# guptakhil/show-tell

Hardware: AMD Instinct MI355X
Metric: training images/sec (ResNet101+GRU, emb=512, bs=128) at 1/2/4/8 MI355X (higher is better)
Workload: dtype bf16; 1 GPU; BASELINE configs[1]: ResNet-101 (train-mode BN, frozen) + 5-layer GRU decoder, E=H=512, V=10000, fwd+bwd+SGD step, synthetic COCO-shaped batch; batch_per_gpu=128, global_batch=128, image=3x224x224, parallelism=dp1

## Files before the change

### include/showtell_hip.h

```cpp
#ifndef SHOWTELL_HIP_H
#define SHOWTELL_HIP_H

#include <stddef.h>
#include <stdint.h>

#ifdef __cplusplus
extern "C" {
#endif

#define ST_F32 0
#define ST_BF16 1

#define ST_CELL_GRU 0
#define ST_CELL_LSTM 1

const char* st_last_error(void);
int st_version(void);

typedef struct {
  const void* x;
  const void* w;
  void* y;
  const float* bias;
  const float* scale;
  const float* shift;
  const void* residual;
  float* stats;
  int dtype, out_dtype;
  int B, Hin, Win, Cin, Ho, Wo, N, KH, KW, stride, pad;
  int ldx, ldw, ldy;
  int relu, accumulate;
  int Cin_logical;
  int k_order;
  int stats_replicas;
  const float* in_stats; const float* in_gamma; const float* in_beta; float in_count, in_eps;
  int split_k;
} st_conv_desc;

int st_conv(const st_conv_desc* d, void* stream);
int st_conv_batch(const st_conv_desc* d, int n, void* stream);

typedef struct {
  const void* x; const void* w_frag; void* y;
  float* stats; int stats_replicas;
  const float* scale; const float* shift; int relu;
  const float* in_stats; const float* in_gamma; const float* in_beta; float in_count; float in_eps;
  int B, H, W, C, N;
  int in_stats_replicas;
} st_conv3x3_img_desc;
int st_conv3x3_img_supported(int H, int W, int C, int N);
int st_conv3x3_img(const st_conv3x3_img_desc* d, void* stream);
int st_conv3x3_s2_supported(int C, int N);
int st_conv3x3_s2(const st_conv3x3_img_desc* d, void* stream);
typedef struct {
  const void* x; const void* w_frag; void* y; const void* residual;
  float* stats; int stats_replicas;
  const float* scale; const float* shift; int relu;
  const float* in_stats; const float* in_gamma; const float* in_beta; float in_count; float in_eps; int in_stats_replicas;
  int B, Hin, Win, C, N, stride;
} st_conv1x1_wreg_desc;
int st_conv1x1_wreg_supported(int C, int N);
int st_conv1x1_wreg(const st_conv1x1_wreg_desc* d, void* stream);
int st_conv1x1_kstream_supported(int C, int N);
int st_conv1x1_kstream(const st_conv1x1_wreg_desc* d, void* stream);
typedef struct {
  const void* raw; const void* identity; void* x_out; const void* w_frag; void* y;
  float* stats; int stats_replicas;
  const float* f_stats; const float* f_gamma; const float* f_beta; float f_count; float f_eps; int f_stats_replicas;
  long rows; int C, N;
  const float* id_stats; const float* id_gamma; const float* id_beta; int id_stats_replicas;
} st_conv1x1_kfuse_desc;
int st_conv1x1_kfuse_supported(int C, int N);
int st_conv1x1_kfuse(const st_conv1x1_kfuse_desc* d, void* stream);
#ifdef ST_EXPERIMENTAL
int st_conv1x1_kfuse8(const st_conv1x1_kfuse_desc* d, void* stream);
#endif
typedef struct {
  const void* raw2; const void* w3_frag; const void* identity; void* x_out; const void* w1_frag; void* y;
  float* stats; int stats_replicas;
  const float* bn2_stats; const float* bn2_gamma; const float* bn2_beta; int bn2_replicas;
  const float* bn3_stats; const float* bn3_gamma; const float* bn3_beta; int bn3_replicas;
  const float* id_stats; const float* id_gamma; const float* id_beta; int id_replicas;
  float count; float eps;
  long rows; int C1, C2, N;
} st_conv_b2b_desc;
int st_conv_b2b_supported(int C1, int C2, int N);
int st_conv_b2b(const st_conv_b2b_desc* d, void* stream);
typedef struct {
  const void* x2; const void* w3_frag; const void* identity; void* x_out; const void* w1_frag; void* y;
  float* stats; int stats_replicas;
  const float* bn2_stats; const float* bn2_gamma; const float* bn2_beta; int bn2_replicas;
  const float* bn3_stats; const float* bn3_gamma; const float* bn3_beta; int bn3_replicas;
  float count; float eps;
  const float* scale3; const float* shift3; const float* scale1; const float* shift1; int relu1;
  long rows; int C1, C2, N;
  const float* id_stats; const float* id_gamma; const float* id_beta; int id_replicas;
} st_conv_c3c1_desc;
int st_conv_c3c1_supported(int C1, int C2, int N);
int st_conv_c3c1(const st_conv_c3c1_desc* d, void* stream);
int st_conv1x1_astat_supported(int C, int N);
int st_conv1x1_astat(const st_conv1x1_wreg_desc* d, void* stream);

int st_pack_conv_weight_frag(const float* w, void* out, int Cout, int Cin, int KH, int KW, int ntw, void* stream);

int st_tune(int reserved, int kc, int w8);
int st_prof_enable(int on);
int st_debug_stamps(unsigned long long* buf);
int st_prof_collect(double* ms, double* flops, long* launches);

typedef struct {
  const void* x; void* y; const void* res;
  const float* stats;  const float* gamma; const float* beta;
  const float* running_mean; const float* running_var;
  const float* res_stats; const float* res_gamma; const float* res_beta;
  const float* res_running_mean; const float* res_running_var;
  int res_bn;
  int dtype; long rows; int C; float count; float eps; int relu;
  int stats_replicas, res_stats_replicas;
} st_bn_act_desc;

int st_bn_act(const st_bn_act_desc* d, void* stream);

int st_bn_update_running(const float* stats, float* running_mean, float* running_var,
// ... 288 lines not shown
```

### show-tell_amd/_lib.py

```python
import ctypes as C
import os

import torch

_HERE = os.path.dirname(os.path.abspath(__file__))
LIB_PATH = os.path.join(_HERE, "lib", "libshowtell_hip.so")

ST_F32, ST_BF16 = 0, 1
ST_CELL_GRU, ST_CELL_LSTM = 0, 1

c_p, c_i, c_f, c_l = C.c_void_p, C.c_int, C.c_float, C.c_long


class ConvDesc(C.Structure):
    _fields_ = [("x", c_p), ("w", c_p), ("y", c_p), ("bias", c_p), ("scale", c_p), ("shift", c_p),
                ("residual", c_p), ("stats", c_p), ("dtype", c_i), ("out_dtype", c_i),
                ("B", c_i), ("Hin", c_i), ("Win", c_i), ("Cin", c_i), ("Ho", c_i), ("Wo", c_i), ("N", c_i),
                ("KH", c_i), ("KW", c_i), ("stride", c_i), ("pad", c_i),
                ("ldx", c_i), ("ldw", c_i), ("ldy", c_i), ("relu", c_i), ("accumulate", c_i), ("Cin_logical", c_i), ("k_order", c_i), ("stats_replicas", c_i),
                ("in_stats", c_p), ("in_gamma", c_p), ("in_beta", c_p), ("in_count", c_f), ("in_eps", c_f), ("split_k", c_i)]


class Conv3x3ImgDesc(C.Structure):
    _fields_ = [("x", c_p), ("w_frag", c_p), ("y", c_p), ("stats", c_p), ("stats_replicas", c_i), ("scale", c_p), ("shift", c_p),
# ... 8 lines not shown


class Conv1x1KfuseDesc(C.Structure):
    _fields_ = [("raw", c_p), ("identity", c_p), ("x_out", c_p), ("w_frag", c_p), ("y", c_p), ("stats", c_p), ("stats_replicas", c_i),
                ("f_stats", c_p), ("f_gamma", c_p), ("f_beta", c_p), ("f_count", c_f), ("f_eps", c_f), ("f_stats_replicas", c_i),
                ("rows", c_l), ("C", c_i), ("N", c_i),
                ("id_stats", c_p), ("id_gamma", c_p), ("id_beta", c_p), ("id_stats_replicas", c_i)]


class StemConvPoolDesc(C.Structure):
    _fields_ = [("x_s2d", c_p), ("w_frag", c_p), ("y", c_p), ("stats", c_p), ("stats_replicas", c_i), ("gamma", c_p),
                ("scale", c_p), ("shift", c_p), ("B", c_i), ("H", c_i), ("W", c_i)]


class ConvB2bDesc(C.Structure):
    _fields_ = [("raw2", c_p), ("w3_frag", c_p), ("identity", c_p), ("x_out", c_p), ("w1_frag", c_p), ("y", c_p),
                ("stats", c_p), ("stats_replicas", c_i),
                ("bn2_stats", c_p), ("bn2_gamma", c_p), ("bn2_beta", c_p), ("bn2_replicas", c_i),
                ("bn3_stats", c_p), ("bn3_gamma", c_p), ("bn3_beta", c_p), ("bn3_replicas", c_i),
                ("id_stats", c_p), ("id_gamma", c_p), ("id_beta", c_p), ("id_replicas", c_i),
                ("count", c_f), ("eps", c_f), ("rows", c_l), ("C1", c_i), ("C2", c_i), ("N", c_i)]


class ConvC3c1Desc(C.Structure):
    _fields_ = [("x2", c_p), ("w3_frag", c_p), ("identity", c_p), ("x_out", c_p), ("w1_frag", c_p), ("y", c_p),
                ("stats", c_p), ("stats_replicas", c_i),
                ("bn2_stats", c_p), ("bn2_gamma", c_p), ("bn2_beta", c_p), ("bn2_replicas", c_i),
                ("bn3_stats", c_p), ("bn3_gamma", c_p), ("bn3_beta", c_p), ("bn3_replicas", c_i),
                ("count", c_f), ("eps", c_f),
                ("scale3", c_p), ("shift3", c_p), ("scale1", c_p), ("shift1", c_p), ("relu1", c_i),
                ("rows", c_l), ("C1", c_i), ("C2", c_i), ("N", c_i),
                ("id_stats", c_p), ("id_gamma", c_p), ("id_beta", c_p), ("id_replicas", c_i)]


class BnActDesc(C.Structure):
    _fields_ = [("x", c_p), ("y", c_p), ("res", c_p), ("stats", c_p), ("gamma", c_p), ("beta", c_p),
                ("running_mean", c_p), ("running_var", c_p), ("res_stats", c_p), ("res_gamma", c_p),
                ("res_beta", c_p), ("res_running_mean", c_p), ("res_running_var", c_p), ("res_bn", c_i),
                ("dtype", c_i), ("rows", c_l), ("C", c_i), ("count", c_f), ("eps", c_f), ("relu", c_i),
                ("stats_replicas", c_i), ("res_stats_replicas", c_i)]


ST_MAX_LAYERS = 8


class RnnParams(C.Structure):
    _fields_ = [("cell", c_i), ("dtype", c_i), ("L", c_i), ("in0", c_i), ("H", c_i), ("V", c_i), ("E", c_i),
                ("emb", c_p), ("w_ih", c_p * ST_MAX_LAYERS), ("w_hh", c_p * ST_MAX_LAYERS),
                ("b_ih", c_p * ST_MAX_LAYERS), ("b_hh", c_p * ST_MAX_LAYERS), ("w_lin", c_p), ("b_lin", c_p)]


class RnnGrads(C.Structure):
    _fields_ = [("emb", c_p), ("w_ih", c_p * ST_MAX_LAYERS), ("w_hh", c_p * ST_MAX_LAYERS),
                ("b_ih", c_p * ST_MAX_LAYERS), ("b_hh", c_p * ST_MAX_LAYERS), ("w_lin", c_p), ("b_lin", c_p)]


class AttnParams(C.Structure):
    _fields_ = [("rnn", RnnParams), ("F", c_i), ("A", c_i), ("P", c_i),
                ("w_enc", c_p), ("b_enc", c_p), ("w_dec", c_p), ("b_dec", c_p), ("w_full", c_p), ("b_full", c_p),
                ("w_init_h", c_p), ("b_init_h", c_p), ("w_init_c", c_p), ("b_init_c", c_p), ("w_embed", c_p), ("b_embed", c_p)]


class AttnGrads(C.Structure):
    _fields_ = [("rnn", RnnGrads)] + [(n, c_p) for n in ("w_enc", "b_enc", "w_dec", "b_dec", "w_full", "b_full", "w_init_h", "b_init_h",
                                                        "w_init_c", "b_init_c", "w_embed", "b_embed")]


class PackedSeq(C.Structure):
    _fields_ = [("B", c_i), ("T", c_i), ("ntok", c_i), ("Tcap", c_i), ("batch_sizes_host", C.POINTER(c_i)),
                ("rows_b", c_p), ("rows_t", c_p), ("prev_row", c_p), ("caption", c_p)]


class ImageBatchDesc(C.Structure):
    _fields_ = [("src", c_p), ("src_bytes", C.c_int64), ("offset", c_p), ("height", c_p), ("width", c_p), ("flip", c_p), ("batch", c_i),
                ("max_height", c_i), ("max_width", c_i), ("out_h", c_i), ("out_w", c_i), ("lut", c_p), ("tmp", c_p),
                ("out", c_p), ("out_u8", c_p)]


_SIGS = {
    "st_version": ([], c_i),
    "st_image_transform": ([C.POINTER(ImageBatchDesc), c_p], c_i),
    "st_conv": ([C.POINTER(ConvDesc), c_p], c_i),
    "st_conv_batch": ([C.POINTER(ConvDesc), c_i, c_p], c_i),
    "st_conv3x3_img_supported": ([c_i, c_i, c_i, c_i], c_i),
    "st_conv3x3_img": ([C.POINTER(Conv3x3ImgDesc), c_p], c_i),
    "st_conv3x3_s2_supported": ([c_i, c_i], c_i),
    "st_conv3x3_s2": ([C.POINTER(Conv3x3ImgDesc), c_p], c_i),
    "st_conv1x1_wreg_supported": ([c_i, c_i], c_i),
    "st_conv1x1_wreg": ([C.POINTER(Conv1x1WregDesc), c_p], c_i),
    "st_conv1x1_kfuse": ([C.POINTER(Conv1x1KfuseDesc), c_p], c_i),
    "st_conv1x1_kfuse_supported": ([c_i, c_i], c_i),
    "st_conv1x1_kfuse8": ([C.POINTER(Conv1x1KfuseDesc), c_p], c_i),
    "st_conv_b2b": ([C.POINTER(ConvB2bDesc), c_p], c_i),
    "st_conv_b2b_supported": ([c_i, c_i, c_i], c_i),
    "st_conv_c3c1": ([C.POINTER(ConvC3c1Desc), c_p], c_i),
    "st_conv_c3c1_supported": ([c_i, c_i, c_i], c_i),
    "st_conv1x1_astat_supported": ([c_i, c_i], c_i),
    "st_conv1x1_astat": ([C.POINTER(Conv1x1WregDesc), c_p], c_i),
    "st_conv1x1_kstream_supported": ([c_i, c_i], c_i),
    "st_conv1x1_kstream": ([C.POINTER(Conv1x1WregDesc), c_p], c_i),
    "st_pack_conv_weight_frag": ([c_p, c_p, c_i, c_i, c_i, c_i, c_i, c_p], c_i),
    "st_tune": ([c_i, c_i, c_i], c_i),
    "st_prof_enable": ([c_i], c_i),
    "st_debug_stamps": ([c_p], c_i),
    "st_prof_collect": ([C.POINTER(C.c_double), C.POINTER(C.c_double), C.POINTER(c_l)], c_i),
    "st_bn_act": ([C.POINTER(BnActDesc), c_p], c_i),
    "st_bn_update_running": ([c_p, c_p, c_p, c_i, c_f, c_f, c_p], c_i),
    "st_nchw_to_nhwc": ([c_p, c_p, c_i, c_i, c_i, c_i, c_i, c_i, c_p], c_i),
    "st_nchw_to_s2d16": ([c_p, c_p, c_i, c_i, c_i, c_i, c_p], c_i),
    "st_stem_weight_s2d": ([c_p, c_p, c_i, c_i, c_p], c_i),
    "st_stem_weight_frag": ([c_p, c_p, c_p], c_i),
    "st_stem_weight_frag_packed": ([c_p, c_i, c_p, c_p], c_i),
    "st_stem_conv_pool": ([C.POINTER(StemConvPoolDesc), c_p], c_i),
    "st_nhwc_to_ncp_f32": ([c_p, c_p, c_i, c_i, c_i, c_i, c_p], c_i),
    "st_maxpool3x3s2": ([c_p, c_p, c_i, c_i, c_i, c_i, c_i, c_p], c_i),
    "st_maxpool3x3s2_bn": ([c_p, c_p, c_i, c_i, c_i, c_i, c_i, c_p, c_p, c_p, c_p, c_p, c_f, c_f, c_p], c_i),
    "st_global_avgpool": ([c_p, c_p, c_i, c_i, c_i, c_i, c_i, c_p], c_i),
    "st_cast": ([c_p, c_p, c_i, c_i, c_l, c_p], c_i),
    "st_transpose": ([c_p, c_p, c_i, c_i, c_i, c_i, c_i, c_p], c_i),
    "st_transpose_colsum": ([c_p, c_p, c_p, c_i, c_i, c_i, c_i, c_i, c_p], c_i),
    "st_transpose_batch": ([c_p, c_p, c_p, c_i, c_i, c_i, c_i, c_i, c_i, c_p, c_p, c_p], c_i),
    "st_pack_conv_weight": ([c_p, c_p, c_i, c_i, c_i, c_i, c_i, c_i, c_i, c_p], c_i),
    "st_cast2d": ([c_p, c_p, c_i, c_i, c_i, c_i, c_i, c_i, c_p], c_i),
    "st_rnn_vocab_ld": ([c_i], c_i),
    "st_rnn_workspace_bytes": ([C.POINTER(RnnParams), C.POINTER(PackedSeq)], C.c_size_t),
    "st_rnn_forward": ([C.POINTER(RnnParams), C.POINTER(PackedSeq), c_p, c_p, c_p, C.c_size_t, c_p, c_i, c_i, c_p, c_i, c_p], c_i),
    "st_rnn_fused_loss_supported": ([C.POINTER(RnnParams)], c_i),
    "st_rnn_fused_loss_bytes": ([C.POINTER(RnnParams), C.POINTER(PackedSeq)], C.c_size_t),
    "st_rnn_fused_loss": ([C.POINTER(RnnParams), C.POINTER(PackedSeq), c_p, C.c_size_t, c_p, c_p, C.c_size_t, c_p, c_p], c_i),
    "st_rnn_fused_dlogits": ([C.POINTER(RnnParams), C.POINTER(PackedSeq), c_p, C.c_size_t, c_p, c_p, c_p, c_p, c_i, c_p], c_i),
    "st_rnn_fused_loss_w": ([C.POINTER(RnnParams), C.POINTER(PackedSeq), c_p, C.c_size_t, c_p, c_p, C.c_size_t, c_p, c_p, c_p, c_p], c_i),
    "st_rnn_fused_dlogits_w": ([C.POINTER(RnnParams), C.POINTER(PackedSeq), c_p, C.c_size_t, c_p, c_p, c_p, c_p, c_p, c_i, c_p], c_i),
    "st_rnn_fused_loss_ls_bytes": ([C.POINTER(RnnParams), C.POINTER(PackedSeq)], C.c_size_t),
    "st_rnn_fused_loss_ls": ([C.POINTER(RnnParams), C.POINTER(PackedSeq), c_p, C.c_size_t, c_p, c_p, C.c_size_t, c_p, c_p, c_p, c_f, c_p,
                             C.c_size_t, c_p, c_p], c_i),
    "st_rnn_fused_dlogits_ls": ([C.POINTER(RnnParams), C.POINTER(PackedSeq), c_p, C.c_size_t, c_p, c_p, c_p, c_p, c_f, c_p, c_i, c_p], c_i),
    "st_rnn_backward": ([C.POINTER(RnnParams), C.POINTER(RnnGrads), C.POINTER(PackedSeq), c_p, c_p, c_i, c_p, c_p, C.c_size_t,
                         c_p, c_p, c_p], c_i),
    "st_dropout_rows": ([c_p, c_p, c_i, c_i, c_i, c_i, c_i, C.c_double, c_l, c_i, c_i, c_i, c_p], c_i),
    "st_rnn_dropout_bytes": ([C.POINTER(RnnParams), C.POINTER(PackedSeq)], C.c_size_t),
    "st_rnn_forward_drop": ([C.POINTER(RnnParams), C.POINTER(PackedSeq), c_p, c_p, c_p, C.c_size_t, c_p, c_i, c_i, c_p, c_i, c_p, c_p], c_i),
    "st_rnn_fused_loss_drop": ([C.POINTER(RnnParams), C.POINTER(PackedSeq), c_p, C.c_size_t, c_p, c_p, C.c_size_t, c_p, c_p, c_p, c_f, c_p,
                               C.c_size_t, c_p, c_p, c_p], c_i),
    "st_rnn_fused_dlogits_drop": ([C.POINTER(RnnParams), C.POINTER(PackedSeq), c_p, C.c_size_t, c_p, c_p, c_p, c_p, c_f, c_p, c_i, c_p, c_p],
                                  c_i),
    "st_rnn_backward_drop": ([C.POINTER(RnnParams), C.POINTER(RnnGrads), C.POINTER(PackedSeq), c_p, c_p, c_i, c_p, c_p, C.c_size_t,
                              c_p, c_p, c_p, c_p], c_i),
    "st_rnn_forward_ids": ([C.POINTER(RnnParams), C.POINTER(PackedSeq), c_p, c_p, c_p, C.c_size_t, c_p, c_i, c_i, c_p, c_i, c_p, c_p, c_p], c_i),
    "st_rnn_backward_ids": ([C.POINTER(RnnParams), C.POINTER(RnnGrads), C.POINTER(PackedSeq), c_p, c_p, c_i, c_p, c_p, C.c_size_t,
                             c_p, c_p, c_p, c_p, c_p], c_i),
    "st_rnn_greedy_workspace_bytes": ([C.POINTER(RnnParams), c_i], C.c_size_t),
    "st_rnn_greedy": ([C.POINTER(RnnParams), c_p, c_i, c_i, c_p, C.c_size_t, c_p, c_p, c_p], c_i),
    "st_rnn_greedy_last_route": ([], c_i),
    "st_rnn_step": ([C.POINTER(RnnParams), c_p, c_i, c_p, c_p, c_p, c_p, c_p, c_i, c_p], c_i),
    "st_embedding_rows": ([c_p, c_p, c_p, c_i, c_i, c_i, c_i, c_i, c_p], c_i),
    "st_gather_state": ([c_p, c_p, c_p, c_i, c_i, c_i, c_i, c_i, c_p], c_i),
    "st_softmax_topk": ([c_p, c_i, c_i, c_i, c_i, c_p, c_p, c_i, c_p], c_i),
    "st_beam_select": ([c_p, c_p, c_p, c_p, c_p, c_i, c_i, c_i, c_l, c_p, c_p, c_p, c_p, c_p, c_p], c_i),
    "st_beam_ban_topk": ([c_p, c_i, c_i, c_i, c_i, c_p, c_i, c_i, c_i, c_p, c_i, c_l, c_i, c_p, c_p, c_p], c_i),
    "st_beam_select_hist": ([c_p, c_p, c_p, c_p, c_p, c_i, c_i, c_i, c_l, c_p, c_p, c_p, c_p, c_p, c_p, c_p, c_i, c_i, c_p], c_i),
    "st_sample_rows": ([c_p, c_i, c_i, c_i, c_p, c_i, c_f, c_i, c_l, c_p, c_p, c_p, c_i, c_i, c_p, c_p], c_i),
    "st_rnn_sample_workspace_bytes": ([C.POINTER(RnnParams), c_i], C.c_size_t),
    "st_rnn_sample": ([C.POINTER(RnnParams), c_p, c_i, c_i, c_p, c_f, c_i, c_l, c_p, C.c_size_t, c_p, c_p, c_p], c_i),
    "st_sample_mix_rows": ([c_p, c_i, c_i, c_i, c_p, c_i, c_f, c_i, c_p, c_i, c_f, c_p, c_i, c_l, c_p, c_i, c_p, c_p, c_p, c_p, c_i, c_i, c_p,
                            c_p], c_i),
    "st_rnn_sched_inputs_workspace_bytes": ([C.POINTER(RnnParams), c_i], C.c_size_t),
# ... 115 lines not shown
```

### show-tell_amd/csrc/rnn.cpp

```cpp
#include "decoder_host.h"
#include <stdlib.h>

namespace {

struct Plan {
  int G, GH, Np, Vp, maxw;
  size_t es;
  size_t x0, y, gates, cst, dyl, dx0, dgx, dgh, dhc, dcc, tA, tB, wT, wThh, wTih, gA, gB, total;
};

Plan make_plan(const st_rnn_params* p, const st_packed_seq* s) {
  Plan q;
  q.G = p->cell == ST_CELL_GRU ? 3 : 4;
  q.GH = q.G * p->H;
  q.Np = st_up8(s->ntok);
  q.Vp = st_rnn_vocab_ld(p->V);
  q.es = st_dtype_size(p->dtype);
  q.maxw = p->in0 > p->H ? p->in0 : p->H;
  const size_t n = s->ntok, L = p->L, H = p->H;
  Arena ar;
  q.x0 = ar.take(n * p->in0 * q.es);
  q.y = ar.take(L * n * H * q.es);
  q.gates = ar.take(L * n * 4 * H * q.es);
  q.cst = ar.take(p->cell == ST_CELL_LSTM ? L * n * H * q.es : 0);
// ... 184 lines not shown
  const char* ytop = reinterpret_cast<const char*>(workspace) + q.y + (size_t)(p->L - 1) * s->ntok * p->H * q.es;
  const int n = s->ntok;
  return vocab_ce_forward(ytop, p->w_lin, p->b_lin, targets, n, p->V, scratch + 2 * (size_t)n, scratch + n, scratch, loss_accum,
                          row_weight, nll_out, reinterpret_cast<hipStream_t>(stream), tile_sums, smooth_out, label_smoothing);
}
extern "C" int st_rnn_fused_dlogits_ls(const st_rnn_params* p, const st_packed_seq* s, const void* workspace, size_t workspace_bytes,
                                       const long* targets, const float* scratch, const float* grad_scale_dev, const float* row_weight,
                                       float label_smoothing, void* dlogits, int ldd, void* stream) {
  if (check_common(p, s, "st_rnn_fused_dlogits_ls")) return 1;
  ST_CHECK(workspace && targets && scratch && dlogits, "st_rnn_fused_dlogits_ls: null pointer");
  ST_CHECK(label_smoothing >= 0.f && label_smoothing < 1.f, "st_rnn_fused_dlogits_ls: label_smoothing=%g outside [0, 1)", (double)label_smoothing);
  ST_CHECK(st_rnn_fused_loss_supported(p), "st_rnn_fused_dlogits_ls: unsupported configuration");
  const Plan q = make_plan(p, s);
  ST_CHECK(workspace_bytes >= q.total, "st_rnn_fused_dlogits_ls: workspace too small");
  const char* ytop = reinterpret_cast<const char*>(workspace) + q.y + (size_t)(p->L - 1) * s->ntok * p->H * q.es;
  return vocab_ce_dlogits(ytop, p->w_lin, p->b_lin, targets, scratch, s->ntok, p->V, dlogits, ldd, 1.0f, grad_scale_dev, row_weight,
                          reinterpret_cast<hipStream_t>(stream), true, label_smoothing);
}

namespace {
int fused_rows(const st_rnn_params* p, const st_packed_seq* s, const void* workspace, size_t workspace_bytes, const st_dropout* drop,
               const char* who, const char** ytop) {
  if (check_common(p, s, who)) return 1;
  ST_CHECK(st_rnn_fused_loss_supported(p), "%s: needs bf16, H = 512 and the vocabulary projection", who);
  const Plan q = make_plan(p, s);
  ST_CHECK(workspace && workspace_bytes >= q.total, "%s: workspace too small", who);
  DropPlan dp;
  if (st_drop_plan(drop, p->L, s->ntok, p->H, p->dtype, false, who, &dp)) return 1;
  *ytop = dp.out ? dp.rows(p->L - 1) : reinterpret_cast<const char*>(workspace) + q.y + (size_t)(p->L - 1) * s->ntok * p->H * q.es;
  return 0;
}
}
extern "C" int st_rnn_fused_loss_drop(const st_rnn_params* p, const st_packed_seq* s, const void* workspace, size_t workspace_bytes,
                                      const long* targets, float* scratch, size_t scratch_bytes, const float* row_weight, float* nll_out,
                                      float* smooth_out, float label_smoothing, float* tile_sums, size_t tile_sums_bytes, float* loss_accum,
                                      const st_dropout* drop, void* stream) {
  const char* ytop;
  if (fused_rows(p, s, workspace, workspace_bytes, drop, "st_rnn_fused_loss_drop", &ytop)) return 1;
  ST_CHECK(targets && scratch && (loss_accum || nll_out || smooth_out), "st_rnn_fused_loss_drop: null pointer");
  ST_CHECK(label_smoothing >= 0.f && label_smoothing < 1.f, "st_rnn_fused_loss_drop: label_smoothing=%g outside [0, 1)", (double)label_smoothing);
  ST_CHECK(scratch_bytes >= st_rnn_fused_loss_bytes(p, s), "st_rnn_fused_loss_drop: scratch too small");
  const int n = s->ntok;
  hipStream_t st = reinterpret_cast<hipStream_t>(stream);
  if (label_smoothing == 0.f && !smooth_out)
    return vocab_ce_forward(ytop, p->w_lin, p->b_lin, targets, n, p->V, scratch + 2 * (size_t)n, scratch + n, scratch, loss_accum, row_weight,
                            nll_out, st);
  ST_CHECK(tile_sums && tile_sums_bytes >= st_rnn_fused_loss_ls_bytes(p, s), "st_rnn_fused_loss_drop: tile_sums too small");
  return vocab_ce_forward(ytop, p->w_lin, p->b_lin, targets, n, p->V, scratch + 2 * (size_t)n, scratch + n, scratch, loss_accum, row_weight,
                          nll_out, st, tile_sums, smooth_out, label_smoothing);
}
extern "C" int st_rnn_fused_dlogits_drop(const st_rnn_params* p, const st_packed_seq* s, const void* workspace, size_t workspace_bytes,
                                         const long* targets, const float* scratch, const float* grad_scale_dev, const float* row_weight,
                                         float label_smoothing, void* dlogits, int ldd, const st_dropout* drop, void* stream) {
  const char* ytop;
  if (fused_rows(p, s, workspace, workspace_bytes, drop, "st_rnn_fused_dlogits_drop", &ytop)) return 1;
  ST_CHECK(targets && scratch && dlogits, "st_rnn_fused_dlogits_drop: null pointer");
  ST_CHECK(label_smoothing >= 0.f && label_smoothing < 1.f, "st_rnn_fused_dlogits_drop: label_smoothing=%g outside [0, 1)", (double)label_smoothing);
  return vocab_ce_dlogits(ytop, p->w_lin, p->b_lin, targets, scratch, s->ntok, p->V, dlogits, ldd, 1.0f, grad_scale_dev, row_weight,
                          reinterpret_cast<hipStream_t>(stream), label_smoothing != 0.f, label_smoothing);
}

namespace {
int rnn_backward(const st_rnn_params* p, const st_rnn_grads* g, const st_packed_seq* s,
                 const void* x0_override, const void* dlogits, int ldd, const float* dy_top_extra,
                 void* workspace, size_t workspace_bytes, float* dfeat, float* dx0_out, const st_dropout* drop, const long* input_ids, void* stream) {
  if (check_common(p, s, "st_rnn_backward")) return 1;
  ST_CHECK(g && workspace, "st_rnn_backward: null pointer");
  DropPlan dp;
  if (st_drop_plan(drop, p->L, s->ntok, p->H, p->dtype, false, "st_rnn_backward", &dp)) return 1;
  ST_CHECK(!(dp.in && x0_override), "st_rnn_backward: input dropout needs the call's own x0 rows (no x0_override)");
  ST_CHECK(!(dp.out && !dlogits), "st_rnn_backward: p_out masks the gradient of the vocabulary projection (needs dlogits, not dy_top)");
  const Plan q = make_plan(p, s);
  ST_CHECK(workspace_bytes >= q.total, "st_rnn_backward: workspace too small (%zu < %zu)", workspace_bytes, q.total);
  hipStream_t st = reinterpret_cast<hipStream_t>(stream);
  char* ws = reinterpret_cast<char*>(workspace);
  const int dt = p->dtype, H = p->H, n = s->ntok, Np = q.Np, GH = q.GH;
  const size_t es = q.es;
  const std::vector<int> off = st_packed_offsets(s);
  const int L = p->L, T = s->T;
  auto dyl = [&](int l) { return reinterpret_cast<float*>(ws + q.dyl) + (size_t)l * n * H; };
  float* dy = dyl(L - 1);
  const char* ytop = dp.out ? dp.rows(L - 1) : ws + q.y + (size_t)(p->L - 1) * n * H * es;

  if (dlogits) {
    ST_CHECK(p->w_lin && g->w_lin && g->b_lin, "st_rnn_backward: vocabulary projection gradients requested without buffers");
    ST_CHECK(ldd >= st_up8(p->V) && ldd % 8 == 0 && ldd <= q.Vp, "st_rnn_backward: dlogits leading dimension %d must be a multiple of 8 in [%d, %d]",
             ldd, st_up8(p->V), q.Vp);
    if (st_transpose_colsum(dlogits, ws + q.tA, g->b_lin, dt, n, p->V, ldd, Np, stream)) return 1;
    if (st_transpose(ytop, ws + q.tB, dt, n, H, H, Np, stream)) return 1;
    if (st_gemm_nt(ws + q.tA, Np, ws + q.tB, Np, g->w_lin, H, p->V, H, Np, dt, ST_F32, nullptr, stream, 1)) return 1;
    if (st_transpose(p->w_lin, ws + q.wT, dt, p->V, H, H, ldd, stream)) return 1;
    const int bk = dt == ST_BF16 ? 64 : 32;
    const int split = (ldd % (8 * bk) == 0 && ldd >= 16 * bk) ? 8 : 0;
    if (st_gemm_nt(dlogits, ldd, ws + q.wT, ldd, dy, H, n, H, ldd, dt, ST_F32, nullptr, stream, 0, split)) return 1;
    if (dy_top_extra) { st_set_error("st_rnn_backward: dlogits and dy_top_extra are exclusive"); return 1; }
    if (dp.out && dropout_rows_launch(dy, dy, ST_F32, n, H, H, H, dp.kout, L - 1, 0, st)) return 1;
  } else {
    ST_CHECK(dy_top_extra, "st_rnn_backward: need dlogits or dy_top");
    if (hipMemcpyAsync(dy, dy_top_extra, (size_t)n * H * sizeof(float), hipMemcpyDeviceToDevice, st) != hipSuccess) {
      st_set_error("st_rnn_backward: copy failed"); return 1;
    }
  }

  const void* x0 = x0_override ? x0_override : ws + q.x0;
  const bool need_dx0 = dfeat || dx0_out || g->emb;
  float* dx0 = dx0_out ? dx0_out : reinterpret_cast<float*>(ws + q.dx0);
  const bool gru = p->cell == ST_CELL_GRU;
  auto dgxl = [&](int l) { return ws + q.dgx + (size_t)l * n * GH * es; };
  auto dghl = [&](int l) { return gru ? ws + q.dgh + (size_t)l * n * GH * es : dgxl(l); };
  auto dhcl = [&](int l) { return reinterpret_cast<float*>(ws + q.dhc) + (size_t)l * s->B * H; };
  auto dccl = [&](int l) { return reinterpret_cast<float*>(ws + q.dcc) + (size_t)l * s->B * H; };
  auto wThh = [&](int l) { return ws + q.wThh + (size_t)l * H * GH * es; };
  auto wTih = [&](int l) { return ws + q.wTih + (size_t)l * q.maxw * GH * es; };
  if (hipMemsetAsync(ws + q.dhc, 0, (size_t)L * s->B * H * sizeof(float), st) != hipSuccess ||
      hipMemsetAsync(ws + q.dcc, 0, (size_t)L * s->B * H * sizeof(float), st) != hipSuccess) { st_set_error("memset failed"); return 1; }
  {
    const void* wx[2][ST_MAX_LAYERS]; void* wy[2][ST_MAX_LAYERS];
    int ni = 0;
    for (int l = 0; l < L; ++l) {
      const int in = l == 0 ? p->in0 : H;
      wx[0][l] = p->w_hh[l]; wy[0][l] = wThh(l);
      if (!(l > 0 || need_dx0)) continue;
      if (in == H) { wx[1][ni] = p->w_ih[l]; wy[1][ni] = wTih(l); ++ni; }
      else if (st_transpose(p->w_ih[l], wTih(l), dt, GH, in, in, GH, stream)) return 1;
    }
    if (st_transpose_batch(wx[0], wy[0], nullptr, L, dt, GH, H, H, GH, nullptr, nullptr, stream)) return 1;
    if (ni && st_transpose_batch(wx[1], wy[1], nullptr, ni, dt, GH, H, H, GH, nullptr, nullptr, stream)) return 1;
  }
  auto bwd_cell = [&](int l, int t, const float* dyrows) {
    const char* yl = ws + q.y + (size_t)l * n * H * es;
    const char* gl = ws + q.gates + (size_t)l * n * 4 * H * es;
    const char* cl = ws + q.cst + (size_t)l * n * H * es;
    RnnBwdCell c;
    memset(&c, 0, sizeof(c));
    c.dy = dyrows ? dyrows + (size_t)off[t] * H : nullptr; c.dhc = dhcl(l); c.dcc = dccl(l);
    c.cache = gl + (size_t)off[t] * 4 * H * es;
    c.hprev = t > 0 ? yl + (size_t)off[t - 1] * H * es : nullptr;
    c.cnew = cl + (size_t)off[t] * H * es;
    c.cprev = t > 0 ? cl + (size_t)off[t - 1] * H * es : nullptr;
    c.dgx = dgxl(l) + (size_t)off[t] * GH * es; c.dgh = dghl(l) + (size_t)off[t] * GH * es; c.Bt = s->batch_sizes_host[t];
    return c;
  };
  const char* env = getenv("ST_BPTT_FUSED");
  const bool fused = !(env && env[0] == '0') || dp.layer;
  for (int d = T + L - 2; fused && d >= 0; --d) {
    RnnBwdFused fc[ST_MAX_LAYERS];
    RnnDropArgs da;
    memset(&da, 0, sizeof(da));
    da.key = dp.klayer;
    int nf = 0;
    for (int l = d < T ? 0 : d - (T - 1); l <= d && l < L; ++l) {
      const int t = d - l;
      RnnBwdFused& f = fc[nf++];
      memset(&f, 0, sizeof(f));
      f.e = bwd_cell(l, t, l == L - 1 ? dy : nullptr);
      da.site[nf - 1] = l; da.row0[nf - 1] = off[t];
      RnnGemmArgs& a = f.g;
      a.M = f.e.Bt; a.N = H;
      if (t + 1 < T) {
        a.A = dghl(l) + (size_t)off[t + 1] * GH * es; a.W = wThh(l); a.M2 = s->batch_sizes_host[t + 1]; a.K = GH; a.lda = GH; a.ldw = GH;
      }
      if (l + 1 < L) {
        a.A2 = dgxl(l + 1) + (size_t)off[t] * GH * es; a.W2 = wTih(l + 1); a.K2 = GH; a.lda2 = GH; a.ldw2 = GH;
      }
    }
    if (dp.layer ? rnn_bwd_fused_launch_batch_drop(fc, nf, p->cell, dt, da, st) : rnn_bwd_fused_launch_batch(fc, nf, p->cell, dt, st)) return 1;
  }
  if (fused && need_dx0 && st_gemm_nt(dgxl(0), GH, wTih(0), GH, dx0, p->in0, n, p->in0, GH, dt, ST_F32, nullptr, stream)) return 1;
  for (int d = T + L - 2; !fused && d >= 0; --d) {
    RnnBwdCell gc[ST_MAX_LAYERS];
    RnnGemmArgs mc[2 * ST_MAX_LAYERS];
    int ng = 0, nm = 0;
    for (int l = d < T ? 0 : d - (T - 1); l <= d && l < L; ++l) {
      const int t = d - l;
      const int bt = s->batch_sizes_host[t];
      const int in = l == 0 ? p->in0 : H;
      gc[ng++] = bwd_cell(l, t, dyl(l));
      if (t > 0) {
        RnnGemmArgs& a = mc[nm++];
        memset(&a, 0, sizeof(a));
        a.A = dghl(l) + (size_t)off[t] * GH * es; a.W = wThh(l); a.M = bt; a.N = H; a.K = GH; a.lda = GH; a.ldw = GH;
        a.out_f32 = dhcl(l); a.ldo = H; a.accumulate = 1;
      }
      if (l > 0 || need_dx0) {
        RnnGemmArgs& a = mc[nm++];
        memset(&a, 0, sizeof(a));
        a.A = dgxl(l) + (size_t)off[t] * GH * es; a.W = wTih(l); a.M = bt; a.N = in; a.K = GH; a.lda = GH; a.ldw = GH;
        a.out_f32 = (l > 0 ? dyl(l - 1) + (size_t)off[t] * H : dx0 + (size_t)off[t] * in); a.ldo = in;
      }
    }
    if (rnn_bwd_gates_launch_batch(gc, ng, H, p->cell, dt, st)) return 1;
    if (rnn_gemm_launch_batch(mc, nm, dt, 0, 0, st)) return 1;
  }
  if (dp.in && need_dx0 && dropout_rows_launch(dx0, dx0, ST_F32, n, p->in0, p->in0, p->in0, dp.kin, kDropSiteInput, 0, st)) return 1;
  st_conv_desc gd[2 * ST_MAX_LAYERS];
  int ng = 0;
  auto wgrad = [&](const void* aT, const void* bT, float* dw, int rows, int cols) {
    gd[ng++] = st_gemm_nt_desc(aT, Np, bT, Np, dw, cols, rows, cols, Np, dt, ST_F32, nullptr, 1);
  };
  const void* tx[4][ST_MAX_LAYERS]; void* ty[4][ST_MAX_LAYERS]; float* tc[4][ST_MAX_LAYERS];
  int nx = 0;
  for (int l = 0; l < L; ++l) {
    const int in = l == 0 ? p->in0 : H;
    const char* xl = l == 0 ? reinterpret_cast<const char*>(x0) : dp.layer ? dp.rows(l - 1) : ws + q.y + (size_t)(l - 1) * n * H * es;
    char* aIh = ws + q.gA + (size_t)(2 * l) * GH * Np * es;
    char* aHh = ws + q.gA + (size_t)(2 * l + 1) * GH * Np * es;
    char* bIh = ws + q.gB + (size_t)(2 * l) * q.maxw * Np * es;
    char* bHh = ws + q.gB + (size_t)(2 * l + 1) * q.maxw * Np * es;
    tx[0][l] = dgxl(l); ty[0][l] = aIh; tc[0][l] = g->b_ih[l];
    tx[2][l] = dghl(l); ty[2][l] = aHh; tc[2][l] = g->b_hh[l];
    tx[3][l] = ws + q.y + (size_t)l * n * H * es; ty[3][l] = bHh; tc[3][l] = nullptr;
    if (in == H) {
      tx[1][nx] = xl; ty[1][nx] = bIh; tc[1][nx] = nullptr; ++nx;
      wgrad(aIh, bIh, g->w_ih[l], GH, in);
    } else {
      if (st_transpose(xl, bIh, dt, n, in, in, Np, stream)) return 1;
    }
    wgrad(gru ? aHh : aIh, bHh, g->w_hh[l], GH, H);
    if (!gru && colsum_launch(dghl(l), g->b_hh[l], n, GH, GH, dt, st)) return 1;
  }
  if (st_transpose_batch(tx[0], ty[0], tc[0], L, dt, n, GH, GH, Np, nullptr, nullptr, stream)) return 1;
  if (nx && st_transpose_batch(tx[1], ty[1], nullptr, nx, dt, n, H, H, Np, nullptr, nullptr, stream)) return 1;
  if (gru && st_transpose_batch(tx[2], ty[2], tc[2], L, dt, n, GH, GH, Np, nullptr, nullptr, stream)) return 1;
  if (st_transpose_batch(tx[3], ty[3], nullptr, L, dt, n, H, H, Np, s->rows_t, s->prev_row, stream)) return 1;
  for (int l = 0; l < L; ++l) {
    const int in = l == 0 ? p->in0 : H;
    if (in != H && st_gemm_nt(ws + q.gA + (size_t)(2 * l) * GH * Np * es, Np, ws + q.gB + (size_t)(2 * l) * q.maxw * Np * es, Np,
                              g->w_ih[l], in, GH, in, Np, dt, ST_F32, nullptr, stream, 1)) return 1;
  }
  for (int i = 0; i < ng; i += 12) {
    if (st_conv_batch(gd + i, ng - i < 12 ? ng - i : 12, stream)) return 1;
  }
  if (need_dx0 && !x0_override) {
    ST_CHECK(g->emb, "st_rnn_backward: embedding gradient buffer missing");
    if (embedding_bwd_launch(dx0, input_ids ? input_ids : s->caption, s->Tcap, s->rows_b, s->rows_t, dfeat, g->emb, n, p->E, p->V, 0, st)) return 1;
  }
  return 0;
}
}

extern "C" int st_rnn_backward(const st_rnn_params* p, const st_rnn_grads* g, const st_packed_seq* s,
                               const void* x0_override, const void* dlogits, int ldd, const float* dy_top_extra,
                               void* workspace, size_t workspace_bytes, float* dfeat, float* dx0_out, void* stream) {
  return rnn_backward(p, g, s, x0_override, dlogits, ldd, dy_top_extra, workspace, workspace_bytes, dfeat, dx0_out, nullptr, nullptr, stream);
}
extern "C" int st_rnn_backward_drop(const st_rnn_params* p, const st_rnn_grads* g, const st_packed_seq* s,
                                    const void* x0_override, const void* dlogits, int ldd, const float* dy_top_extra,
                                    void* workspace, size_t workspace_bytes, float* dfeat, float* dx0_out, const st_dropout* drop,
                                    void* stream) {
  return rnn_backward(p, g, s, x0_override, dlogits, ldd, dy_top_extra, workspace, workspace_bytes, dfeat, dx0_out, drop, nullptr, stream);
}
extern "C" int st_rnn_backward_ids(const st_rnn_params* p, const st_rnn_grads* g, const st_packed_seq* s,
                                   const void* x0_override, const void* dlogits, int ldd, const float* dy_top_extra,
                                   void* workspace, size_t workspace_bytes, float* dfeat, float* dx0_out, const st_dropout* drop,
                                   const long* input_ids, void* stream) {
  ST_CHECK(!(input_ids && x0_override), "st_rnn_backward_ids: input_ids and x0_override are exclusive");
  return rnn_backward(p, g, s, x0_override, dlogits, ldd, dy_top_extra, workspace, workspace_bytes, dfeat, dx0_out, drop, input_ids, stream);
}
```

Before: 32310 images/sec.

## Add batched TN GEMM for RNN weight gradients, skipping explicit transposes

Adds a grouped bf16 GEMM kernel that computes C += A^T B directly from row-major activations and gradients. It transposes in LDS with ds_read_tr, gathers previous-step hidden rows by index, and folds the bias column sums into the same pass. The decoder backward uses it by default for the vocabulary projection and all GRU layer weight gradients, replacing separate transpose/colsum kernels and the conv-based wgrad batch. This is meant to remove extra transpose memory traffic and kernel launches. The embedding backward is moved ahead of these GEMMs.

```diff
diff --git a/include/showtell_hip.h b/include/showtell_hip.h
--- a/include/showtell_hip.h
+++ b/include/showtell_hip.h
@@ -39,6 +39,21 @@
 
 int st_conv(const st_conv_desc* d, void* stream);
 int st_conv_batch(const st_conv_desc* d, int n, void* stream);
+
+typedef struct {
+  const void* a;
+  const void* b;
+  float* c;
+  const int* b_row;
+  const int* b_live;
+  float* colsum0;
+  float* colsum1;
+  int dtype;
+  int M, N, K;
+  int lda, ldb, ldc;
+  int accumulate;
+} st_gemm_tn_desc;
+int st_gemm_tn_batch(const st_gemm_tn_desc* d, int n, void* stream);
 
 typedef struct {
   const void* x; const void* w_frag; void* y;
diff --git a/show-tell_amd/_lib.py b/show-tell_amd/_lib.py
--- a/show-tell_amd/_lib.py
+++ b/show-tell_amd/_lib.py
@@ -114,6 +114,7 @@
     "st_image_transform": ([C.POINTER(ImageBatchDesc), c_p], c_i),
     "st_conv": ([C.POINTER(ConvDesc), c_p], c_i),
     "st_conv_batch": ([C.POINTER(ConvDesc), c_i, c_p], c_i),
+    "st_gemm_tn_batch": ([c_p, c_i, c_p], c_i),
     "st_conv3x3_img_supported": ([c_i, c_i, c_i, c_i], c_i),
     "st_conv3x3_img": ([C.POINTER(Conv3x3ImgDesc), c_p], c_i),
     "st_conv3x3_s2_supported": ([c_i, c_i], c_i),
diff --git a/show-tell_amd/csrc/gemm_tn.hip b/show-tell_amd/csrc/gemm_tn.hip
--- /dev/null
+++ b/show-tell_amd/csrc/gemm_tn.hip
@@ -0,0 +1,217 @@
+#include "common.h"
+#include "tn_tile.h"
+#include <string.h>
+#include <type_traits>
+
+namespace {
+
+constexpr int kMaxGroups = 12;
+constexpr int kImages = 2;
+constexpr int kStep = kImages * TN_BK;
+constexpr int kRowsPerThread = kStep / 16;
+
+struct TnGroup {
+  const bf16_t* a; const bf16_t* b; float* c;
+  const int* b_row; const int* b_live;
+  float* cs0; float* cs1;
+  int M, N, K, lda, ldb, ldc, accumulate;
+  int tile0, ntn;
+};
+struct TnArgs { TnGroup g[kMaxGroups]; int ng, ntiles; };
+
+typedef __attribute__((ext_vector_type(4))) short s16x4;
+typedef __attribute__((ext_vector_type(8))) short s16x8;
+typedef __attribute__((address_space(3))) s16x4 lds_s16x4;
+
+__device__ __forceinline__ bf16x8 tr_frag(const char* image, int lane, int c16) {
+  const s16x4 lo = __builtin_amdgcn_ds_read_tr16_b64_v4i16((lds_s16x4*)(image + tn_read_off(lane, c16, 0)));
+  const s16x4 hi = __builtin_amdgcn_ds_read_tr16_b64_v4i16((lds_s16x4*)(image + tn_read_off(lane, c16, 1)));
+  const s16x8 v = __builtin_shufflevector(lo, hi, 0, 1, 2, 3, 4, 5, 6, 7);
+  return *reinterpret_cast<const bf16x8*>(&v);
+}
+
+__global__ __launch_bounds__(256, 2) void gemm_tn_kernel(TnArgs args) {
+  __shared__ __attribute__((aligned(16))) char lds[2][2][kImages][TN_IMAGE_BYTES];
+
+  const int per = gridDim.x >> 3;
+  const int tile = (blockIdx.x & 7) * per + (blockIdx.x >> 3);
+  if (tile >= args.ntiles) return;
+  int gi = 0;
+  while (gi + 1 < args.ng && tile >= args.g[gi + 1].tile0) ++gi;
+  const TnGroup& g = args.g[gi];
+  const int local = tile - g.tile0;
+  const int m0 = (local / g.ntn) * TN_COLS, n0 = (local % g.ntn) * TN_COLS;
+  const int M = g.M, N = g.N, K = g.K;
+  const long lda = g.lda, ldb = g.ldb;
+
+  const int tid = threadIdx.x, lane = tid & 63, wave = tid >> 6;
+  const int ch = tid & 15, r0 = tid >> 4;
+  const bool a_ok = m0 + 8 * ch < M, b_ok = n0 + 8 * ch < N;
+  const bf16_t* ap = g.a + m0 + 8 * ch;
+  const bf16_t* bp = g.b + n0 + 8 * ch;
+  const int* b_row = g.b_row; const int* b_live = g.b_live;
+  const bool do_cs = n0 == 0 && (g.cs0 || g.cs1);
+
+  u32x4 ra[kRowsPerThread], rb[kRowsPerThread];
+  int idx[kRowsPerThread], live[kRowsPerThread];
+  auto resolve = [&](int kbase) {
+    if (!b_row) return;
+#pragma unroll
+    for (int i = 0; i < kRowsPerThread; ++i) {
+      const int k = kbase + r0 + 16 * i, kk = k < K ? k : K - 1;
+      idx[i] = b_row[kk];
+      live[i] = 1;
+    }
+    if (b_live) {
+#pragma unroll
+      for (int i = 0; i < kRowsPerThread; ++i) {
+        const int k = kbase + r0 + 16 * i;
+        live[i] = b_live[k < K ? k : K - 1];
+      }
+    }
+  };
+  auto load = [&](int kbase) {
+#pragma unroll
+    for (int i = 0; i < kRowsPerThread; ++i) {
+      const int k = kbase + r0 + 16 * i;
+      int src = k;
+      if (b_row) src = live[i] > 0 ? idx[i] : -1;
+      ra[i] = u32x4{0u, 0u, 0u, 0u}; rb[i] = u32x4{0u, 0u, 0u, 0u};
+      if (a_ok && k < K) ra[i] = *reinterpret_cast<const u32x4*>(ap + k * lda);
+      if (b_ok && k < K && src >= 0) rb[i] = *reinterpret_cast<const u32x4*>(bp + src * ldb);
+    }
+  };
+
+  f32x4 acc[4][4];
+#pragma unroll
+  for (int i = 0; i < 4; ++i)
+#pragma unroll
+    for (int j = 0; j < 4; ++j) acc[i][j] = f32x4{0.f, 0.f, 0.f, 0.f};
+  float cs[8];
+#pragma unroll
+  for (int e = 0; e < 8; ++e) cs[e] = 0.f;
+
+  const int wm = wave >> 1, wn = wave & 1;
+  const int nsteps = (K + kStep - 1) / kStep;
+  resolve(0);
+  load(0);
+  resolve(kStep);
+  for (int s = 0; s < nsteps; ++s) {
+    char* buf = &lds[s & 1][0][0][0];
+#pragma unroll
+    for (int i = 0; i < kRowsPerThread; ++i) {
+      const int row = r0 + 16 * i;
+      const int off = (row / TN_BK) * TN_IMAGE_BYTES + tn_store_off(row % TN_BK, ch);
+      *reinterpret_cast<u32x4*>(buf + off) = ra[i];
+      *reinterpret_cast<u32x4*>(buf + kImages * TN_IMAGE_BYTES + off) = rb[i];
+    }
+    if (do_cs) {
+#pragma unroll
+      for (int i = 0; i < kRowsPerThread; ++i)
+#pragma unroll
+        for (int e = 0; e < 4; ++e) {
+          cs[2 * e] += __uint_as_float(ra[i][e] << 16);
+          cs[2 * e + 1] += __uint_as_float(ra[i][e] & 0xffff0000u);
+        }
+    }
+    __syncthreads();
+    if (s + 1 < nsteps) {
+      load((s + 1) * kStep);
+      resolve((s + 2) * kStep);
+    }
+#pragma unroll
+    for (int im = 0; im < kImages; ++im) {
+      const char* ia = buf + im * TN_IMAGE_BYTES;
+      const char* ib = buf + (kImages + im) * TN_IMAGE_BYTES;
+      bf16x8 fa[4], fb[4];
+#pragma unroll
+      for (int i = 0; i < 4; ++i) { fa[i] = tr_frag(ia, lane, 4 * wm + i); fb[i] = tr_frag(ib, lane, 4 * wn + i); }
+#pragma unroll
+      for (int i = 0; i < 4; ++i)
+#pragma unroll
+        for (int j = 0; j < 4; ++j) acc[i][j] = __builtin_amdgcn_mfma_f32_16x16x32_bf16(fa[i], fb[j], acc[i][j], 0, 0, 0);
+    }
+  }
+
+  float* const cbase = g.c;
+  const long ldc = g.ldc;
+  const bool accumulate = g.accumulate != 0;
+  auto write_c = [&](auto full_tag) {
+    constexpr bool kFull = decltype(full_tag)::value;
+    float* const cl = cbase + (long)(m0 + 64 * wm + 4 * (lane >> 4)) * ldc + (n0 + 64 * wn + (lane & 15));
+#pragma unroll
+    for (int i0 = 0; i0 < 4; i0 += 2) {
+      float prior[2][4][4];
+#pragma unroll
+      for (int i = 0; i < 2; ++i)
+#pragma unroll
+        for (int r = 0; r < 4; ++r)
+#pragma unroll
+          for (int j = 0; j < 4; ++j) {
+            const int m = m0 + 64 * wm + 16 * (i0 + i) + 4 * (lane >> 4) + r, n = n0 + 64 * wn + 16 * j + (lane & 15);
+            const bool ok = kFull || (m < M && n < N);
+            prior[i][r][j] = 0.f;
+            if (accumulate) prior[i][r][j] = ok ? cl[(16 * (i0 + i) + r) * ldc + 16 * j] : 0.f;
+          }
+#pragma unroll
+      for (int i = 0; i < 2; ++i)
+#pragma unroll
+        for (int r = 0; r < 4; ++r)
+#pragma unroll
+          for (int j = 0; j < 4; ++j) {
+            const int m = m0 + 64 * wm + 16 * (i0 + i) + 4 * (lane >> 4) + r, n = n0 + 64 * wn + 16 * j + (lane & 15);
+            if (kFull || (m < M && n < N)) cl[(16 * (i0 + i) + r) * ldc + 16 * j] = prior[i][r][j] + acc[i0 + i][j][r];
+          }
+    }
+  };
+  if (m0 + TN_COLS <= M && n0 + TN_COLS <= N) write_c(std::true_type{});
+  else write_c(std::false_type{});
+
+  if (do_cs) {
+    __syncthreads();
+    float* red = reinterpret_cast<float*>(&lds[0][0][0][0]);
+#pragma unroll
+    for (int e = 0; e < 8; ++e) red[r0 * TN_COLS + 8 * ch + e] = cs[e];
+    __syncthreads();
+    if (tid < TN_COLS && m0 + tid < M) {
+      float sum = 0.f;
+#pragma unroll
+      for (int r = 0; r < 16; ++r) sum += red[r * TN_COLS + tid];
+      if (g.cs0) g.cs0[m0 + tid] += sum;
+      if (g.cs1) g.cs1[m0 + tid] += sum;
+    }
+  }
+}
+
+}
+
+extern "C" int st_gemm_tn_batch(const st_gemm_tn_desc* d, int n, void* stream) {
+  ST_CHECK(d && n >= 1 && n <= kMaxGroups, "st_gemm_tn_batch: 1..%d problems per launch", kMaxGroups);
+  TnArgs args;
+  memset(&args, 0, sizeof(args));
+  long tiles = 0;
+  for (int i = 0; i < n; ++i) {
+    const st_gemm_tn_desc& p = d[i];
+    ST_CHECK(p.dtype == ST_BF16, "st_gemm_tn_batch: problem %d: bf16 only (the transposed LDS read is a 16-bit one)", i);
+    ST_CHECK(p.a && p.b && p.c, "st_gemm_tn_batch: problem %d: null pointer", i);
+    ST_CHECK(p.M >= 1 && p.N >= 1 && p.K >= 1, "st_gemm_tn_batch: problem %d: bad shape M=%d N=%d K=%d", i, p.M, p.N, p.K);
+    ST_CHECK(p.lda >= p.M && p.ldb >= p.N && p.ldc >= p.N, "st_gemm_tn_batch: problem %d: leading dimension below the extent (lda=%d M=%d ldb=%d N=%d ldc=%d)",
+             i, p.lda, p.M, p.ldb, p.N, p.ldc);
+    ST_CHECK(p.lda % 8 == 0 && p.ldb % 8 == 0, "st_gemm_tn_batch: problem %d: lda=%d and ldb=%d must be multiples of 8", i, p.lda, p.ldb);
+    ST_CHECK(((reinterpret_cast<uintptr_t>(p.a) | reinterpret_cast<uintptr_t>(p.b)) & 15) == 0, "st_gemm_tn_batch: problem %d: a and b must be 16-byte aligned", i);
+    ST_CHECK(!p.b_live || p.b_row, "st_gemm_tn_batch: problem %d: b_live goes with b_row", i);
+    TnGroup& g = args.g[i];
+    g.a = reinterpret_cast<const bf16_t*>(p.a); g.b = reinterpret_cast<const bf16_t*>(p.b); g.c = p.c;
+    g.b_row = p.b_row; g.b_live = p.b_live; g.cs0 = p.colsum0; g.cs1 = p.colsum1;
+    g.M = p.M; g.N = p.N; g.K = p.K; g.lda = p.lda; g.ldb = p.ldb; g.ldc = p.ldc; g.accumulate = p.accumulate;
+    g.tile0 = (int)tiles;
+    g.ntn = (p.N + TN_COLS - 1) / TN_COLS;
+    tiles += (long)((p.M + TN_COLS - 1) / TN_COLS) * g.ntn;
+    ST_CHECK(tiles < (1L << 24), "st_gemm_tn_batch: too many output tiles");
+  }
+  args.ng = n; args.ntiles = (int)tiles;
+  const int grid = (int)((tiles + 7) / 8 * 8);
+  hipLaunchKernelGGL(gemm_tn_kernel, dim3(grid), dim3(256), 0, reinterpret_cast<hipStream_t>(stream), args);
+  ST_LAUNCH_CHECK();
+  return 0;
+}
diff --git a/show-tell_amd/csrc/rnn.cpp b/show-tell_amd/csrc/rnn.cpp
--- a/show-tell_amd/csrc/rnn.cpp
+++ b/show-tell_amd/csrc/rnn.cpp
@@ -290,13 +290,30 @@
   float* dy = dyl(L - 1);
   const char* ytop = dp.out ? dp.rows(L - 1) : ws + q.y + (size_t)(p->L - 1) * n * H * es;
 
+  const char* env_tn = getenv("ST_WGRAD_TN");
+  const bool tn = dt == ST_BF16 && !(env_tn && env_tn[0] == '0');
+  st_gemm_tn_desc tg[2 * ST_MAX_LAYERS + 1];
+  int ntg = 0;
+  auto tn_desc = [&](const void* a, int lda, const void* b, int ldb, float* c, int rows, int cols, float* cs0, float* cs1, bool hprev) {
+    st_gemm_tn_desc d;
+    memset(&d, 0, sizeof(d));
+    d.a = a; d.b = b; d.c = c; d.colsum0 = cs0; d.colsum1 = cs1; d.dtype = dt;
+    d.M = rows; d.N = cols; d.K = n; d.lda = lda; d.ldb = ldb; d.ldc = cols; d.accumulate = 1;
+    if (hprev) { d.b_row = s->prev_row; d.b_live = s->rows_t; }
+    return d;
+  };
+
   if (dlogits) {
     ST_CHECK(p->w_lin && g->w_lin && g->b_lin, "st_rnn_backward: vocabulary projection gradients requested without buffers");
     ST_CHECK(ldd >= st_up8(p->V) && ldd % 8 == 0 && ldd <= q.Vp, "st_rnn_backward: dlogits leading dimension %d must be a multiple of 8 in [%d, %d]",
              ldd, st_up8(p->V), q.Vp);
-    if (st_transpose_colsum(dlogits, ws + q.tA, g->b_lin, dt, n, p->V, ldd, Np, stream)) return 1;
-    if (st_transpose(ytop, ws + q.tB, dt, n, H, H, Np, stream)) return 1;
-    if (st_gemm_nt(ws + q.tA, Np, ws + q.tB, Np, g->w_lin, H, p->V, H, Np, dt, ST_F32, nullptr, stream, 1)) return 1;
+    if (tn) {
+      tg[ntg++] = tn_desc(dlogits, ldd, ytop, H, g->w_lin, p->V, H, g->b_lin, nullptr, false);
+    } else {
+      if (st_transpose_colsum(dlogits, ws + q.tA, g->b_lin, dt, n, p->V, ldd, Np, stream)) return 1;
+      if (st_transpose(ytop, ws + q.tB, dt, n, H, H, Np, stream)) return 1;
+      if (st_gemm_nt(ws + q.tA, Np, ws + q.tB, Np, g->w_lin, H, p->V, H, Np, dt, ST_F32, nullptr, stream, 1)) return 1;
+    }
     if (st_transpose(p->w_lin, ws + q.wT, dt, p->V, H, H, ldd, stream)) return 1;
     const int bk = dt == ST_BF16 ? 64 : 32;
     const int split = (ldd % (8 * bk) == 0 && ldd >= 16 * bk) ? 8 : 0;
@@ -401,6 +418,20 @@
     if (rnn_gemm_launch_batch(mc, nm, dt, 0, 0, st)) return 1;
   }
   if (dp.in && need_dx0 && dropout_rows_launch(dx0, dx0, ST_F32, n, p->in0, p->in0, p->in0, dp.kin, kDropSiteInput, 0, st)) return 1;
+  if (need_dx0 && !x0_override) {
+    ST_CHECK(g->emb, "st_rnn_backward: embedding gradient buffer missing");
+    if (embedding_bwd_launch(dx0, input_ids ? input_ids : s->caption, s->Tcap, s->rows_b, s->rows_t, dfeat, g->emb, n, p->E, p->V, 0, st)) return 1;
+  }
+  for (int l = 0; tn && l < L; ++l) {
+    const int in = l == 0 ? p->in0 : H;
+    const char* xl = l == 0 ? reinterpret_cast<const char*>(x0) : dp.layer ? dp.rows(l - 1) : ws + q.y + (size_t)(l - 1) * n * H * es;
+    tg[ntg++] = tn_desc(dgxl(l), GH, xl, in, g->w_ih[l], GH, in, g->b_ih[l], gru ? nullptr : g->b_hh[l], false);
+    tg[ntg++] = tn_desc(dghl(l), GH, ws + q.y + (size_t)l * n * H * es, H, g->w_hh[l], GH, H, gru ? g->b_hh[l] : nullptr, nullptr, true);
+  }
+  for (int i = 0; i < ntg; i += 12) {
+    if (st_gemm_tn_batch(tg + i, ntg - i < 12 ? ntg - i : 12, stream)) return 1;
+  }
+  if (tn) return 0;
   st_conv_desc gd[2 * ST_MAX_LAYERS];
   int ng = 0;
   auto wgrad = [&](const void* aT, const void* bT, float* dw, int rows, int cols) {
@@ -439,10 +470,6 @@
   for (int i = 0; i < ng; i += 12) {
     if (st_conv_batch(gd + i, ng - i < 12 ? ng - i : 12, stream)) return 1;
   }
-  if (need_dx0 && !x0_override) {
-    ST_CHECK(g->emb, "st_rnn_backward: embedding gradient buffer missing");
-    if (embedding_bwd_launch(dx0, input_ids ? input_ids : s->caption, s->Tcap, s->rows_b, s->rows_t, dfeat, g->emb, n, p->E, p->V, 0, st)) return 1;
-  }
   return 0;
 }
 }
diff --git a/show-tell_amd/csrc/tn_tile.h b/show-tell_amd/csrc/tn_tile.h
--- /dev/null
+++ b/show-tell_amd/csrc/tn_tile.h
@@ -0,0 +1,23 @@
+#pragma once
+
+#if defined(__HIPCC__) || defined(__CUDACC__)
+#define TN_HD __host__ __device__ __forceinline__
+#else
+#define TN_HD inline
+#endif
+
+constexpr int TN_BK = 32;
+constexpr int TN_COLS = 128;
+constexpr int TN_ROW_BYTES = 2 * TN_COLS;
+constexpr int TN_IMAGE_BYTES = TN_BK * TN_ROW_BYTES;
+
+TN_HD int tn_swz(int row) { return ((row & 3) << 2) | ((row >> 2) & 3); }
+
+TN_HD int tn_store_off(int row, int ch) { return TN_ROW_BYTES * row + 16 * (ch ^ tn_swz(row)); }
+
+TN_HD int tn_read_row(int lane, int h) { return 8 * (lane >> 4) + 4 * h + ((lane & 15) >> 2); }
+
+TN_HD int tn_read_off(int lane, int c16, int h) {
+  const int p = lane & 3;
+  return tn_store_off(tn_read_row(lane, h), 2 * c16 + (p >> 1)) + 8 * (p & 1);
+}
diff --git a/show-tell_amd/gemm_tn.py b/show-tell_amd/gemm_tn.py
--- /dev/null
+++ b/show-tell_amd/gemm_tn.py
@@ -0,0 +1,28 @@
+import ctypes as C
+
+import torch
+
+from ._lib import ST_BF16, ShowTellHipError, check, lib, ptr, stream
+
+c_p, c_i = C.c_void_p, C.c_int
+
+
+class GemmTnDesc(C.Structure):
+    _fields_ = [("a", c_p), ("b", c_p), ("c", c_p), ("b_row", c_p), ("b_live", c_p), ("colsum0", c_p), ("colsum1", c_p),
+                ("dtype", c_i), ("M", c_i), ("N", c_i), ("K", c_i), ("lda", c_i), ("ldb", c_i), ("ldc", c_i), ("accumulate", c_i)]
+
+
+def desc(a, b, c, M, N, K=None, b_row=None, b_live=None, colsum0=None, colsum1=None, accumulate=False):
+    for t in (a, b, c):
+        if not t.is_cuda or t.dim() != 2 or t.stride(1) != 1:
+            raise ShowTellHipError("gemm_tn: operands must be 2-d device tensors with unit column stride")
+    if a.dtype != torch.bfloat16 or b.dtype != torch.bfloat16 or c.dtype != torch.float32:
+        raise ShowTellHipError("gemm_tn: a and b are bfloat16, c is float32")
+    return GemmTnDesc(a=ptr(a), b=ptr(b), c=ptr(c), b_row=ptr(b_row), b_live=ptr(b_live), colsum0=ptr(colsum0), colsum1=ptr(colsum1),
+                      dtype=ST_BF16, M=M, N=N, K=a.shape[0] if K is None else K, lda=a.stride(0), ldb=b.stride(0), ldc=c.stride(0),
+                      accumulate=int(bool(accumulate)))
+
+
+def gemm_tn_batch(descs):
+    arr = (GemmTnDesc * max(len(descs), 1))(*descs)
+    check(lib().st_gemm_tn_batch(arr, len(descs), stream()), "st_gemm_tn_batch")
```

Measured after the change: 32730 images/sec (median of 6 runs). 1.3% higher.
